# B3zaleel/draco-sharp

Measured on AMD Instinct MI355X. Metric: decoded_meshes_per_sec, higher is better.
Workload: dtype int32

## Files before the change

### draco-sharp_amd/csrc/dsa_kernels.h

```cpp
#pragma once
#include <hip/hip_runtime.h>
#include <stdint.h>

#include "dsa_common.h"
#include "dsa_locate.h"
#ifdef DSA_EXPERIMENTS
#include "dsa_lanes.h"
#else
#define LN_FLAG_SYMBOLS 1u
#define LN_FLAG_PREDICT 2u
#define LN_FLAG_OCT 8u
namespace dsa { namespace lanes {
__device__ __forceinline__ bool ln_sym_eligible(const AttrDesc &, const MeshLayout &, uint32_t, uint32_t) { return false; }
__device__ __forceinline__ bool ln_oct_eligible(const AttrDesc &, uint32_t) { return false; }
} }
#endif

#ifndef DSA_CHAIN_PRIO
#define DSA_CHAIN_PRIO 3
#endif

namespace dsa {

__device__ __forceinline__ uint32_t cnext(uint32_t c) { return (c % 3u == 2u) ? c - 2u : c + 1u; }
// ... 9 lines not shown
#define SYM_WIDE 0x800u
#define SYM_EARLY_ONLY 0x100u
#define SYM_LATE_ONLY 0x200u
#define SYM_CORNER 0x1000u
#define PRED_FRONT 0x10000u
#define PRED_BEHIND 0x20000u
__device__ __forceinline__ bool att_behind_tables(const AttrDesc &a) { return a.corner_data != 0 || a.late_located != 0; }
__device__ __forceinline__ bool att_is_late(const AttrDesc &a) { return (a.have_scheme && a.pred_kind != 0) || att_behind_tables(a); }
#define PW_FLAG 4u
#define LATE_HANDOFF 0x40000u
__device__ __forceinline__ void late_handoff(uint8_t *arena, const MeshLayout &L, MeshDesc *D, uint32_t ai, uint32_t flags, uint32_t bit);
__device__ __forceinline__ bool pred_filtered(const AttrDesc &a, uint32_t flags) {
  return ((flags & PRED_FRONT) && att_behind_tables(a)) || ((flags & PRED_BEHIND) && !att_behind_tables(a));
}
__device__ __forceinline__ bool sym_filtered(const AttrDesc &a, uint32_t flags) {
  if (att_behind_tables(a)) return !(flags & SYM_CORNER);
  if (flags & SYM_CORNER) return true;
  const bool late = a.have_scheme && a.pred_kind != 0;
  return ((flags & SYM_EARLY_ONLY) && late) || ((flags & SYM_LATE_ONLY) && !late);
}
__device__ __forceinline__ uint64_t clk() { return __builtin_amdgcn_s_memtime(); }
__device__ __forceinline__ uint64_t realclk() { return __builtin_amdgcn_s_memrealtime(); }
__device__ __forceinline__ uint32_t leading_lanes(bool pred) { uint64_t m = ~__ballot(pred); return m ? (uint32_t)__builtin_ctzll(m) : 64u; }
#define WAIT_VM0() __builtin_amdgcn_s_waitcnt(0x0F70)

template <int CTRL>
__device__ __forceinline__ uint32_t dpp_mov(uint32_t x) { return (uint32_t)__builtin_amdgcn_update_dpp(0, (int)x, CTRL, 0xF, 0xF, false); }
__device__ __forceinline__ uint32_t lane_prev(uint32_t x) { return dpp_mov<0x138>(x); }
template <class Op>
__device__ __forceinline__ uint32_t wave_incl_scan(uint32_t x, Op op) {
  const uint32_t lane = lane_id(), rl = lane & 15u;
  uint32_t t;
  t = dpp_mov<0x111>(x); if (rl >= 1) x = op(t, x);
  t = dpp_mov<0x112>(x); if (rl >= 2) x = op(t, x);
  t = dpp_mov<0x114>(x); if (rl >= 4) x = op(t, x);
  t = dpp_mov<0x118>(x); if (rl >= 8) x = op(t, x);
  t = dpp_mov<0x142>(x); if ((lane & 31u) >= 16) x = op(t, x);
  t = dpp_mov<0x143>(x); if (lane >= 32) x = op(t, x);
  return x;
}
__device__ __forceinline__ uint32_t wave_excl_scan(uint32_t v, uint32_t *total) {
  const uint32_t x = wave_incl_scan(v, [](uint32_t a, uint32_t b) { return a + b; });
  *total = rdlane(x, 63);
  return x - v;
}

template <bool CP> struct Rec;
struct FaceIds { uint32_t v0, v1, v2, o0, o1, o2; };
template <> struct Rec<false> {
  static constexpr uint32_t WORDS = 8;
  struct Raw { uint4 v, o; };
  static __device__ __forceinline__ Raw load(const uint32_t *frec, uint32_t f) { Raw r; r.v = ((const uint4 *)frec)[(size_t)f * 2]; r.o = ((const uint4 *)frec)[(size_t)f * 2 + 1]; return r; }
  static __device__ __forceinline__ Raw none() { Raw r; r.v = make_uint4(0, 0, 0, 0); r.o = make_uint4(DSA_INVALID, DSA_INVALID, DSA_INVALID, 0); return r; }
  static __device__ __forceinline__ uint32_t sel3(uint32_t k, uint32_t x, uint32_t y, uint32_t z) { return k == 0 ? x : (k == 1 ? y : z); }
  static __device__ __forceinline__ uint32_t vertex(const Raw &r, uint32_t k) { return sel3(k, r.v.x, r.v.y, r.v.z); }
  static __device__ __forceinline__ uint32_t opp(const Raw &r, uint32_t k) { return sel3(k, r.o.x, r.o.y, r.o.z); }
  static __device__ __forceinline__ uint32_t get_v(const uint32_t *frec, uint32_t c) { return frec[fv_idx(c)]; }
  static __device__ __forceinline__ uint32_t get_o(const uint32_t *frec, uint32_t c) { return frec[fo_idx(c)]; }
  static __device__ __forceinline__ uint32_t get_o_plain(const uint32_t *frec, uint32_t c) { return frec[fo_idx(c)]; }
  static __device__ __forceinline__ void set_v(uint32_t *frec, uint32_t c, uint32_t val) { frec[fv_idx(c)] = val; }
  static __device__ __forceinline__ void link(uint32_t *frec, uint32_t c, uint32_t val) { frec[fo_idx(c)] = val; }
  static __device__ __forceinline__ void link_lds(uint32_t *stage, uint32_t c_rel, uint32_t val) { stage[fo_idx(c_rel)] = val; }
  static __device__ __forceinline__ void store(uint32_t *frec, uint32_t f, const FaceIds &x) {
    ((uint4 *)frec)[(size_t)f * 2] = make_uint4(x.v0, x.v1, x.v2, 0u); ((uint4 *)frec)[(size_t)f * 2 + 1] = make_uint4(x.o0, x.o1, x.o2, 0u);
  }
  static __device__ __forceinline__ void store_lds(uint32_t *stage, uint32_t slot, const FaceIds &x) {
    *(uint4 *)&stage[slot * 8] = make_uint4(x.v0, x.v1, x.v2, 0u); *(uint4 *)&stage[slot * 8 + 4] = make_uint4(x.o0, x.o1, x.o2, 0u);
  }
  static __device__ __forceinline__ uint4 vertices_of(const uint32_t *frec, uint32_t f) { return ((const uint4 *)frec)[(size_t)f * 2]; }
};
template <> struct Rec<true> {
  static constexpr uint32_t WORDS = 4;
  static constexpr uint32_t M = 0x1FFFFFu;
  struct Raw { uint64_t v, o; };
  static __device__ __forceinline__ uint64_t pack(uint32_t a, uint32_t b, uint32_t c) { return (uint64_t)(a & M) | ((uint64_t)(b & M) << 21) | ((uint64_t)(c & M) << 42); }
  static __device__ __forceinline__ uint32_t field(uint64_t w, uint32_t k) { return (uint32_t)((int32_t)((uint32_t)(w >> (21u * k)) << 11) >> 11); }
  static __device__ __forceinline__ Raw load(const uint32_t *frec, uint32_t f) { const uint4 q = ((const uint4 *)frec)[f]; Raw r; r.v = (uint64_t)q.x | ((uint64_t)q.y << 32); r.o = (uint64_t)q.z | ((uint64_t)q.w << 32); return r; }
  static __device__ __forceinline__ Raw none() { Raw r; r.v = 0; r.o = ~0ull; return r; }
  static __device__ __forceinline__ uint32_t vertex(const Raw &r, uint32_t k) { return field(r.v, k); }
  static __device__ __forceinline__ uint32_t opp(const Raw &r, uint32_t k) { return field(r.o, k); }
  static __device__ __forceinline__ uint32_t get_v(const uint32_t *frec, uint32_t c) { return field(((const uint64_t *)frec)[(size_t)(c >> 2) * 2], c & 3u); }
  static __device__ __forceinline__ uint32_t get_o(const uint32_t *frec, uint32_t c) {
    return field(__hip_atomic_load((const unsigned long long *)frec + (size_t)(c >> 2) * 2 + 1, __ATOMIC_RELAXED, __HIP_MEMORY_SCOPE_AGENT), c & 3u);
  }
  static __device__ __forceinline__ uint32_t get_o_plain(const uint32_t *frec, uint32_t c) { return field(((const uint64_t *)frec)[(size_t)(c >> 2) * 2 + 1], c & 3u); }
  static __device__ __forceinline__ void set_v(uint32_t *frec, uint32_t c, uint32_t val) {
    uint64_t *w = (uint64_t *)frec + (size_t)(c >> 2) * 2;
    const uint32_t sh = 21u * (c & 3u);
    *w = (*w & ~((uint64_t)M << sh)) | ((uint64_t)(val & M) << sh);
  }
  static __device__ __forceinline__ void link(uint32_t *frec, uint32_t c, uint32_t val) {
    const uint32_t sh = 21u * (c & 3u);
    atomicAnd((unsigned long long *)frec + (size_t)(c >> 2) * 2 + 1, ((unsigned long long)(val & M) << sh) | ~((unsigned long long)M << sh));
  }
  static __device__ __forceinline__ void link_lds(uint32_t *stage, uint32_t c_rel, uint32_t val) {
    const uint32_t sh = 21u * (c_rel & 3u);
    atomicAnd((unsigned long long *)stage + (size_t)(c_rel >> 2) * 2 + 1, ((unsigned long long)(val & M) << sh) | ~((unsigned long long)M << sh));
  }
  static __device__ __forceinline__ uint4 quad(const FaceIds &x) { const uint64_t v = pack(x.v0, x.v1, x.v2), o = pack(x.o0, x.o1, x.o2); return make_uint4((uint32_t)v, (uint32_t)(v >> 32), (uint32_t)o, (uint32_t)(o >> 32)); }
  static __device__ __forceinline__ void store(uint32_t *frec, uint32_t f, const FaceIds &x) { ((uint4 *)frec)[f] = quad(x); }
  static __device__ __forceinline__ void store_lds(uint32_t *stage, uint32_t slot, const FaceIds &x) { *(uint4 *)&stage[slot * 4] = quad(x); }
  static __device__ __forceinline__ uint4 vertices_of(const uint32_t *frec, uint32_t f) {
    const uint64_t v = ((const uint64_t *)frec)[(size_t)f * 2];
    return make_uint4(field(v, 0), field(v, 1), field(v, 2), 0u);
  }
};
__device__ __forceinline__ uint32_t k_next(uint32_t k) { return k == 2u ? 0u : k + 1u; }
__device__ __forceinline__ uint32_t k_prev(uint32_t k) { return k == 0u ? 2u : k - 1u; }

__device__ __forceinline__ uint8_t *seam_block(uint8_t *arena, const MeshLayout &L, const SeamLayout &g, uint32_t d) {
  return arena + L.seam + g.data + (uint64_t)d * g.data_stride;
}
__device__ __forceinline__ const uint32_t *att_para(uint8_t *arena, const MeshLayout &L, const MeshDesc *D, const AttrDesc &a) {
  if (a.corner_data == 0) return (const uint32_t *)(arena + L.para);
  const SeamLayout g = seam_layout(L.cap_faces, L.cap_vertices, D->num_att_data, L.rec_compact != 0);
  return (const uint32_t *)(seam_block(arena, L, g, (uint32_t)a.corner_data - 1u) + g.para);
}


template <bool TOGGLE>
__device__ __forceinline__ uint32_t rabs_block_to_words(const Rabs &rb, uint32_t count, uint32_t *words) {
  uint32_t state = rb.state, left = rb.off, first = DSA_INVALID;
  const uint32_t p = rb.p;
  const uintptr_t a0 = (uintptr_t)rb.buf + (left ? left - 1u : 0u);
  const uint32_t *wp = (const uint32_t *)(a0 & ~(uintptr_t)3);
  uint32_t sh = (uint32_t)(a0 & 3u) * 8u;
  uint32_t cur = wp[0], nxt = wp[-1];
  uint32_t word = 0, last = 1;
  for (uint32_t i = 0; i < count; ++i) {
    if (state < 4096u && left > 0u) {
      state = state * 256u + ((cur >> sh) & 255u);
// ... 851 lines not shown
  uint32_t F, NV, cap_entries, expect;
  int att_data;
};
__device__ __forceinline__ TravIO trav_position(uint8_t *arena, const MeshLayout &L, const MeshDesc *D) {
  TravIO io;
  io.frec = (const uint32_t *)(arena + L.frec); io.d2c = (uint32_t *)(arena + L.d2c); io.v2d = (int32_t *)(arena + L.v2d);
  io.fvis = arena + L.fvis; io.vflag = arena + L.vvis; io.stack = (uint32_t *)(arena + L.fstamp); io.para = (uint32_t *)(arena + L.para);
  io.F = D->num_faces; io.NV = D->num_vertices; io.cap_entries = L.cap_vertices; io.expect = D->num_enc_vertices; io.att_data = -1;
  return io;
}
__device__ __forceinline__ TravIO trav_attribute(uint8_t *arena, const MeshLayout &L, const MeshDesc *D, uint32_t d) {
  const SeamLayout g = seam_layout(L.cap_faces, L.cap_vertices, D->num_att_data, L.rec_compact != 0);
  uint8_t *blk = seam_block(arena, L, g, d);
  TravIO io;
  io.frec = (const uint32_t *)(blk + g.rec); io.d2c = (uint32_t *)(blk + g.d2c); io.v2d = (int32_t *)(blk + g.v2d);
  io.fvis = blk + g.fvis; io.vflag = blk + g.vflag; io.stack = (uint32_t *)(blk + g.stack); io.para = (uint32_t *)(blk + g.para);
  io.F = D->num_faces; io.NV = D->seam_nv[d]; io.cap_entries = 3u * L.cap_faces; io.expect = D->seam_nv[d]; io.att_data = (int)d;
  return io;
}
template <bool CP>
__device__ __forceinline__ void traverse_wave(uint8_t *arena, const MeshLayout &L, MeshDesc *D, const TravIO &io, uint32_t fuse_operands, unsigned long long *sh_tf,
                                              unsigned long long *sh_tv, uint32_t *sh_hist) {
  typedef Rec<CP> R;
  typedef typename R::Raw Raw;
  if (status_of(D) != ST_OK || D->encoder_type == 0 || D->general) return;
  const uint32_t *frec = io.frec;
  uint32_t *d2c = io.d2c;
  int32_t *v2d = io.v2d;
  uint8_t *fvis = io.fvis;
  uint8_t *vflag = io.vflag;
  const uint32_t F = uni(io.F), NV = uni(io.NV), cap_entries = uni(io.cap_entries), expect = uni(io.expect);
  const bool position = io.att_data < 0;
  uint32_t *stack = io.stack;
  const uint32_t stack_cap = F;
  const uint32_t lane = lane_id();
  const uint64_t t_start = clk(), r_start = realclk();

  uint32_t count = 0, sp = 0, f_scan = 0;
  uint32_t run_id = 0;
  bool have_prog = false, prog_lin = false;
  uint32_t p_a = 0, p_an = 0, p_b = 0, p_ta = 0, p_tb = 0, p_la = 0, p_rb = 0;
  uint32_t dir = 0, hist_strikes = 0;
  uint32_t backoff = 0;
  uint32_t fail_streak = 0;
  uint32_t window = WAVE, side1 = WAVE, side2 = WAVE;
  uint32_t n_run = 0, n_run_faces = 0, n_scalar = 0, n_fail = 0, n_fast = 0;
  bool failed = false;
  bool have_rec = false, have_state = false, must_scalar = false, have2 = false;
  bool no_hist = false;
  uint32_t c_v = 0, c_rc = 0, c_lc = 0, c_bits = 0;
  uint32_t c2_v = 0, c2_rc = 0, c2_lc = 0, c2_bits = 0;
#ifdef DSA_TRAV_PROFILE
  uint64_t tp_acc[6] = {0, 0, 0, 0, 0, 0}, tp_last = clk();
  uint32_t np_fast_hit = 0, np_dep = 0, np_head = 0, np_hist = 0, np_lin = 0, np_hand = 0;
#define TPROF(slot_) { const uint64_t t_ = clk(); tp_acc[slot_] += t_ - tp_last; tp_last = t_; }
#define TCOUNT(x_) ++x_
#else
#define TPROF(slot_)
#define TCOUNT(x_)
#endif
#define TR_FAIL(site) { if (lane == 0) fail(D, ST_INVALID, (site)); failed = true; break; }
#define VISIT_SCALAR(v_, c_, fl_) { if (lane == 0) { vflag[v_] = (uint8_t)((fl_) | 1u); d2c[count] = (c_); v2d[v_] = (int32_t)count; } ++count; }
  auto corner_ok = [&](uint32_t c) -> bool { return c < 4 * F && (c & 3u) != 3u; };

  for (;;) {
    if (sp == 0) {
      uint32_t found = DSA_INVALID;
      while (f_scan < F) {
        uint32_t f = f_scan + lane;
        uint64_t m = __ballot(f < F && fvis[f] == 0);
        if (m) { found = f_scan + (uint32_t)__builtin_ctzll(m); break; }
        f_scan += WAVE;
      }
      if (found == DSA_INVALID) break;
      f_scan = found;
      const uint32_t corner = 4 * found;
      if (lane == 0) stack[0] = corner;
      sp = 1;
      const uint4 vv = R::vertices_of(frec, found);
      const uint32_t nv = uni(vv.y), pv = uni(vv.z);
      if (nv >= NV || pv >= NV) TR_FAIL(300);
      { uint32_t uni_flag = uni((uint32_t)vflag[nv]); if (!(uni_flag & 1u)) { if (count >= cap_entries) TR_FAIL(302); VISIT_SCALAR(nv, corner + 1, uni_flag); } }
      WAIT_VM0();
      { uint32_t uni_flag = uni((uint32_t)vflag[pv]); if (!(uni_flag & 1u)) { if (count >= cap_entries) TR_FAIL(302); VISIT_SCALAR(pv, corner + 2, uni_flag); } }
      WAIT_VM0();
    }
    uint32_t corner = uni(stack[sp - 1]);
    have_prog = false; have_rec = false; have_state = false; must_scalar = false; have2 = false;
    if (corner == DSA_INVALID || corner >= 4 * F || uni((uint32_t)fvis[corner >> 2])) { --sp; continue; }

    for (;;) {
      uint32_t face = corner >> 2;
      uint32_t v = 0, rc = 0, lc = 0, bits = 0;
      bool have_kids = false;
      uint32_t kr_v = 0, kr_rc = 0, kr_lc = 0, kl_v = 0, kl_rc = 0, kl_lc = 0;
      uint32_t kind = 0;
      bool lin = false;
      (void)lin;
      uint32_t a = 0, b = 0, tipA = 0, lcA = DSA_INVALID, tipB = 0, rcB = DSA_INVALID, lcB = DSA_INVALID;
      uint32_t marks = 0x0000011Eu;
#define fA_before (marks & 1u)
#define fB_before ((marks >> 1) & 1u)
#define fR_before ((marks >> 2) & 1u)
#define fL_before ((marks >> 3) & 1u)
#define fLA_before ((marks >> 4) & 1u)
#define flA ((marks >> 8) & 3u)
#define flB ((marks >> 16) & 3u)
#define TR_MARKS(fa_, fb_, fr_, fl_, fla_, ta_, tb_) (((fa_) ? 1u : 0u) | ((fb_) ? 2u : 0u) | ((fr_) ? 4u : 0u) | ((fl_) ? 8u : 0u) | ((fla_) ? 16u : 0u) | (((ta_) & 3u) << 8) | (((tb_) & 3u) << 16))
      bool pair_ok = false;
      uint32_t len = 0;

      if (have_prog && backoff == 0) { kind = 1; lin = prog_lin; }
      else {
        Raw rb0 = R::none();
        bool have_seed = false;
        if (have_rec) { v = c_v; rc = c_rc; lc = c_lc; }
        else {
          const Raw r0 = R::load(frec, face);
          const uint32_t kc0 = corner & 3u;
          v = uni(R::vertex(r0, kc0)); rc = uni(R::opp(r0, k_next(kc0))); lc = uni(R::opp(r0, k_prev(kc0)));
        }
        if (v >= NV || (rc != DSA_INVALID && !corner_ok(rc)) || (lc != DSA_INVALID && !corner_ok(lc))) TR_FAIL(301);
        if (have_state) bits = c_bits;
        else {
          const uint32_t tip_flag = vflag[v];
          const uint32_t side_r = rc != DSA_INVALID ? (uint32_t)fvis[rc >> 2] : 1u, side_l = lc != DSA_INVALID ? (uint32_t)fvis[lc >> 2] : 1u;
          Raw rl0 = R::none();
          if (rc != DSA_INVALID) { rb0 = R::load(frec, rc >> 2); have_seed = true; }
          if (lc != DSA_INVALID) rl0 = R::load(frec, lc >> 2);
          have_kids = true;
          { const uint32_t kr = rc & 3u, kl = lc & 3u;
            kr_v = uni(R::vertex(rb0, kr)); kr_rc = uni(R::opp(rb0, k_next(kr))); kr_lc = uni(R::opp(rb0, k_prev(kr)));
            kl_v = uni(R::vertex(rl0, kl)); kl_rc = uni(R::opp(rl0, k_next(kl))); kl_lc = uni(R::opp(rl0, k_prev(kl))); }
          const uint32_t uf = uni(tip_flag);
          const bool rdone = rc == DSA_INVALID || (rc >> 2) == face || uni(side_r) != 0;
          const bool ldone = lc == DSA_INVALID || (lc >> 2) == face || uni(side_l) != 0;
          bits = ((uf & 1u) ? 0u : 1u) | (uf & 2u) | (rdone ? 4u : 0u) | (ldone ? 8u : 0u);
          TCOUNT(np_head);
        }
        have_rec = false; have_state = false;
        const bool moves_right = (bits & 3u) == 1u || ((bits & 12u) == 8u);
        if (moves_right && backoff == 0 && !must_scalar && rc != DSA_INVALID) {
          if (!have_seed) rb0 = R::load(frec, rc >> 2);
          const uint32_t kb0 = rc & 3u;
          const uint32_t tB0 = uni(R::vertex(rb0, kb0)), rB0 = uni(R::opp(rb0, k_next(kb0))), a1 = uni(R::opp(rb0, k_prev(kb0)));
          const uint32_t d1 = a1 - corner;
          const uint32_t e = dir & 3u;
          const bool hm = !no_hist && d1 != 0u && corner_ok(a1) && uni(sh_hist[8 * e]) == d1;
          if (hm) {
            const uint32_t s_b = uni(sh_hist[8 * e + 1]), s_ta = uni(sh_hist[8 * e + 2]), s_tb = uni(sh_hist[8 * e + 3]), s_la = uni(sh_hist[8 * e + 4]), s_rb = uni(sh_hist[8 * e + 5]);
            p_a = corner + lane * d1; p_an = p_a + d1; p_b = rc + lane * s_b; p_ta = v + lane * s_ta; p_tb = tB0 + lane * s_tb;
            p_la = lc == DSA_INVALID ? DSA_INVALID : lc + lane * s_la; p_rb = rB0 == DSA_INVALID ? DSA_INVALID : rB0 + lane * s_rb;
            kind = 2; lin = true;
            TCOUNT(np_hist);
          } else {
            kind = 3;
            auto opp_prev_of = [&](uint32_t b1) -> uint32_t { return corner_ok(b1) ? uni(R::get_o_plain(frec, qprev(b1))) : DSA_INVALID; };
            auto opp_next_of = [&](uint32_t c) -> uint32_t { return corner_ok(c) ? uni(R::get_o_plain(frec, qnext(c))) : DSA_INVALID; };
            const uint32_t a0 = corner;
            const uint32_t a2 = opp_prev_of(opp_next_of(a1));
            const uint32_t d2 = a2 - a1, ddh = d2 - d1;
            const uint32_t exact = corner_ok(a2) ? 3u : (corner_ok(a1) ? 2u : 1u);
            uint32_t lq = lane;
            asm volatile("" : "+v"(lq));
            a = lane == 0 ? a0 : lane == 1 ? a1 : lane == 2 ? a2 : a2 + (lane - 2u) * (d2 + ddh) + ddh * ((lq - 2u) * (lq - 3u) / 2u);
            bool a_ok = lane < window && corner_ok(a) && (lane < exact || exact == 3);
            Raw ra = R::none(), rb = R::none();
            if (a_ok) ra = R::load(frec, a >> 2);
            const uint32_t ka = a & 3u;
            tipA = R::vertex(ra, ka); b = R::opp(ra, k_next(ka)); lcA = R::opp(ra, k_prev(ka));
            const bool b_ok = a_ok && corner_ok(b) && tipA < NV && (lcA == DSA_INVALID || corner_ok(lcA));
            if (b_ok) rb = R::load(frec, b >> 2);
            const uint32_t kb = b & 3u;
            tipB = R::vertex(rb, kb); rcB = R::opp(rb, k_next(kb)); lcB = R::opp(rb, k_prev(kb));
            const uint32_t next_a = b_ok ? lcB : DSA_INVALID;
            {
              const uint32_t prev_next = lane_prev(next_a);
              a_ok = a_ok && (lane == 0 || prev_next == a);
            }
            len = leading_lanes(a_ok);
            pair_ok = lane < len && b_ok && tipB < NV && corner_ok(lcB) && (rcB == DSA_INVALID || corner_ok(rcB));
            if (pair_ok) {
              const uint32_t m0 = lane == 0 ? 0u : fvis[a >> 2], m4 = lcA != DSA_INVALID ? fvis[lcA >> 2] : 1u, m1 = fvis[b >> 2];
              const uint32_t m2 = rcB != DSA_INVALID ? fvis[rcB >> 2] : 1u, m3 = fvis[lcB >> 2], ta = vflag[tipA], tb = vflag[tipB];
              marks = TR_MARKS(m0, m1, m2, m3, m4, ta, tb);
            }
            TCOUNT(np_dep);
          }
        } else if (backoff) --backoff;
        must_scalar = false;
        TPROF(1);
      }

      if (kind == 1 || kind == 2) {
        ++n_fast;
        a = p_a;
        const bool a_ok = lane < window && corner_ok(a);
        const bool bp_ok = a_ok && corner_ok(p_b);
        Raw ra = R::none(), rb = R::none();
        if (a_ok) ra = R::load(frec, a >> 2);
        if (bp_ok) rb = R::load(frec, p_b >> 2);
        if (bp_ok) {
          const uint32_t m0 = lane == 0 ? 0u : fvis[a >> 2], m1 = fvis[p_b >> 2], m4 = corner_ok(p_la) ? fvis[p_la >> 2] : 1u;
          const uint32_t m2 = corner_ok(p_rb) ? fvis[p_rb >> 2] : 1u, m3 = corner_ok(p_an) ? fvis[p_an >> 2] : 1u;
          const uint32_t ta = p_ta < NV ? vflag[p_ta] : 1u, tb = p_tb < NV ? vflag[p_tb] : 1u;
          marks = TR_MARKS(m0, m1, m2, m3, m4, ta, tb);
        }
        const uint32_t ka = a & 3u, kb = p_b & 3u;
        tipA = R::vertex(ra, ka); b = R::opp(ra, k_next(ka)); lcA = R::opp(ra, k_prev(ka));
        tipB = R::vertex(rb, kb); rcB = R::opp(rb, k_next(kb)); lcB = R::opp(rb, k_prev(kb));
        const bool match = bp_ok && b == p_b && tipA == p_ta && lcA == p_la && tipB == p_tb && rcB == p_rb && lcB == p_an &&
                           tipA < NV && tipB < NV && corner_ok(lcB) && (lcA == DSA_INVALID || corner_ok(lcA)) && (rcB == DSA_INVALID || corner_ok(rcB));
        len = leading_lanes(match);
        pair_ok = lane < len;
        if (kind == 1) {
          v = rdlane(tipA, 0); rc = rdlane(b, 0); lc = rdlane(lcA, 0);
          if (v >= NV || (rc != DSA_INVALID && !corner_ok(rc)) || (lc != DSA_INVALID && !corner_ok(lc))) TR_FAIL(301);
        }
        TPROF(0);
      } else if (kind == 3) { TPROF(2); }

      if (kind) {
        const uint32_t fa = a >> 2, fb = b >> 2;
        const uint32_t keyN = 2 * lane, keyL = 2 * lane + 1;
        uint32_t sfa = TR_NONE, sfb = TR_NONE, sta = TR_NONE, stb = TR_NONE, srf = TR_NONE, slf = TR_NONE, sla = TR_NONE;
        int32_t fa0, fas, fad, fb0, fbs, fbd, ta0, tas, tad, tb0, tbs, tbd;
        bool arith;
        {
          const uint32_t tri = lane * (lane - 1u) / 2u;
          const bool two = len >= 2, three = len >= 3;
          auto fit = [&](uint32_t x, int32_t &q0, int32_t &qs, int32_t &qd) {
            const uint32_t x0 = rdlane(x, 0), x1 = rdlane(x, 1), x2 = rdlane(x, 2);
            q0 = (int32_t)x0; qs = two ? (int32_t)(x1 - x0) : 1; qd = three ? (int32_t)((x2 - x1) - (x1 - x0)) : 0;
          };
          auto mono = [&](int32_t s_, int32_t d_) -> bool {
            const int32_t last = s_ + d_ * (int32_t)(two ? len - 2u : 0u);
            return s_ != 0 && last != 0 && ((s_ ^ last) >= 0) && d_ > -(1 << 24) && d_ < (1 << 24);
          };
          int32_t a0, as_, ad, b0, bs_, bd;
          fit(a, a0, as_, ad); fit(b, b0, bs_, bd); fit(tipA, ta0, tas, tad); fit(tipB, tb0, tbs, tbd);
          arith = ((as_ | ad | bs_ | bd) & 3) == 0 && mono(as_, ad) && mono(bs_, bd) && mono(tas, tad) && mono(tbs, tbd);
          if (arith && kind == 3)
            arith = __ballot(lane < len && (a != (uint32_t)a0 + lane * (uint32_t)as_ + (uint32_t)ad * tri || b != (uint32_t)b0 + lane * (uint32_t)bs_ + (uint32_t)bd * tri ||
                                            tipA != (uint32_t)ta0 + lane * (uint32_t)tas + (uint32_t)tad * tri || tipB != (uint32_t)tb0 + lane * (uint32_t)tbs + (uint32_t)tbd * tri)) == 0;
          fa0 = a0 >> 2; fas = as_ >> 2; fad = ad >> 2; fb0 = b0 >> 2; fbs = bs_ >> 2; fbd = bd >> 2;
        }
        if (arith) {
          TCOUNT(np_lin);
          const float iA = 1.0f / (float)fas, iB = 1.0f / (float)fbs, iTA = 1.0f / (float)tas, iTB = 1.0f / (float)tbs;
          auto pos_in = [&](uint32_t X, int32_t first, int32_t step, int32_t dd, float inv, uint32_t odd) -> uint32_t {
            if (dd == 0) {
              const int32_t d = (int32_t)X - first;
              const int32_t j = (int32_t)__builtin_rintf((float)d * inv);
              return (j >= 0 && (uint32_t)j < len && j * step == d) ? 2u * (uint32_t)j + odd : TR_NONE;
            }
            int32_t j = 0;
#pragma unroll
            for (int32_t bit = 32; bit >= 1; bit >>= 1) {
              const int32_t t = j + bit;
              const int32_t qt = first + t * step + dd * (t * (t - 1) / 2);
              if ((uint32_t)t < len && (step > 0 ? qt <= (int32_t)X : qt >= (int32_t)X)) j = t;
            }
            return first + j * step + dd * (j * (j - 1) / 2) == (int32_t)X ? 2u * (uint32_t)j + odd : TR_NONE;
          };
          auto face_pos = [&](uint32_t X) -> uint32_t { const uint32_t x = pos_in(X, fa0, fas, fad, iA, 0u), y = pos_in(X, fb0, fbs, fbd, iB, 1u); return x < y ? x : y; };
          auto tip_pos = [&](uint32_t X) -> uint32_t { const uint32_t x = pos_in(X, ta0, tas, tad, iTA, 0u), y = pos_in(X, tb0, tbs, tbd, iTB, 1u); return x < y ? x : y; };
          if (pair_ok) {
            sfa = face_pos(fa); sfb = face_pos(fb);
            if (!(flA & 1u)) sta = tip_pos(tipA);
            if (!(flB & 1u)) stb = tip_pos(tipB);
            if (rcB != DSA_INVALID && fR_before == 0) srf = face_pos(rcB >> 2);
            if (fL_before == 0) slf = face_pos(lcB >> 2);
            if (lcA != DSA_INVALID && fLA_before == 0 && flA != 0) sla = face_pos(lcA >> 2);
          }
        } else {
          if (++run_id >= 0x00FFFFF0u) {
            __syncthreads();
            for (uint32_t i = lane; i < TR_SLOTS; i += WAVE) { sh_tf[i] = 0; sh_tv[i] = 0; }
            __syncthreads();
            run_id = 1;
          }
          const uint32_t run_tag = 0x00FFFFFFu - run_id;
          auto tbl_insert = [&](unsigned long long *t, uint32_t id, uint32_t pos) {
            const unsigned long long want = ((unsigned long long)run_tag << 40) | ((unsigned long long)id << 8) | pos;
            uint32_t sl = (id * 2654435761u) >> (32 - TR_SLOT_BITS);
            for (;;) {
              const unsigned long long cur = __hip_atomic_load(&t[sl], __ATOMIC_RELAXED, __HIP_MEMORY_SCOPE_WORKGROUP);
              if ((uint32_t)(cur >> 40) != run_tag) { if (atomicCAS(&t[sl], cur, want) == cur) break; continue; }
              if ((uint32_t)(cur >> 8) == id) { atomicMin(&t[sl], want); break; }
              sl = (sl + 1) & (TR_SLOTS - 1);
            }
          };
          auto tbl_lookup = [&](unsigned long long *t, uint32_t id) -> uint32_t {
            uint32_t sl = (id * 2654435761u) >> (32 - TR_SLOT_BITS);
            for (uint32_t probes = 0; probes < TR_SLOTS; ++probes) {
              const unsigned long long cur = __hip_atomic_load(&t[sl], __ATOMIC_RELAXED, __HIP_MEMORY_SCOPE_WORKGROUP);
              if ((uint32_t)(cur >> 40) != run_tag) return TR_NONE;
              if ((uint32_t)(cur >> 8) == id) return (uint32_t)(cur & 0xFFu);
              sl = (sl + 1) & (TR_SLOTS - 1);
            }
            return TR_NONE;
          };
          if (pair_ok) {
            tbl_insert(sh_tf, fa, 2 * lane); tbl_insert(sh_tf, fb, 2 * lane + 1);
            if (!(flA & 1u)) tbl_insert(sh_tv, tipA, 2 * lane);
            if (!(flB & 1u)) tbl_insert(sh_tv, tipB, 2 * lane + 1);
          }
          __syncthreads();
          if (pair_ok) {
            sfa = tbl_lookup(sh_tf, fa); sfb = tbl_lookup(sh_tf, fb);
            if (!(flA & 1u)) sta = tbl_lookup(sh_tv, tipA);
            if (!(flB & 1u)) stb = tbl_lookup(sh_tv, tipB);
            if (rcB != DSA_INVALID && fR_before == 0) srf = tbl_lookup(sh_tf, rcB >> 2);
            if (fL_before == 0) slf = tbl_lookup(sh_tf, lcB >> 2);
            if (lcA != DSA_INVALID && fLA_before == 0 && flA != 0) sla = tbl_lookup(sh_tf, lcA >> 2);
          }
        }
        bool good = false, newA = false, newB = false;
        uint32_t hand = 0;
        if (pair_ok) {
          newA = !(flA & 1u) && sta == keyN;
          const bool la_done = lcA == DSA_INVALID || (lcA >> 2) == fa || fLA_before != 0 || sla < keyN;
          const bool x_ok = fA_before == 0 && sfa == keyN && ((newA && !(flA & 2u)) || la_done);
          newB = !(flB & 1u) && stb == keyL;
          const bool r_done = rcB == DSA_INVALID || (rcB >> 2) == fb || fR_before != 0 || srf < keyL;
          const bool l_open = (lcB >> 2) != fb && fL_before == 0 && !(slf < keyL);
          const bool y_ok = fB_before == 0 && sfb == keyL && !(newB && !(flB & 2u)) && r_done && l_open;
          good = x_ok && y_ok;
// ... 12 lines not shown
        TPROF(3);
        const uint64_t kmask = K >= 64 ? ~0ull : ((1ull << K) - 1ull);
        const uint64_t mA = __ballot(newA) & kmask, mB = __ballot(newB) & kmask;
        const uint32_t made = (uint32_t)__popcll(mA) + (uint32_t)__popcll(mB);
        const bool retire = K >= 1 && count + made <= cap_entries;
        const uint32_t win_used = window;
        have_prog = false;
        if (kind == 2) {
          if (K == len && len <= 2 && len < window) { if (++hist_strikes >= 2) { if (lane == 0) sh_hist[8 * (dir & 3u)] = 0; hist_strikes = 0; } }
          else if (K >= 3) hist_strikes = 0;
        }
        if (retire) {
          if (lane < K) {
            const uint64_t lt = (1ull << lane) - 1ull;
            const uint32_t posA = count + (uint32_t)__popcll(mA & lt) + (uint32_t)__popcll(mB & lt);
            fvis[fa] = 1; fvis[fb] = 1;
            if (newA) { vflag[tipA] = (uint8_t)(flA | 1u); d2c[posA] = a; v2d[tipA] = (int32_t)posA; }
            if (newB) { const uint32_t posB = posA + (newA ? 1u : 0u); vflag[tipB] = (uint8_t)(flB | 1u); d2c[posB] = b; v2d[tipB] = (int32_t)posB; }
          }
          const uint32_t nxt = rdlane(lcB, K - 1);
          count += made;
          if (K >= 3) {
            const uint32_t aK1 = rdlane(a, K - 1), aK2 = rdlane(a, K - 2), aK3 = rdlane(a, K - 3);
            const uint32_t s1 = nxt - aK1, s0 = aK1 - aK2, sm = aK2 - aK3;
            const uint32_t a_d = (s1 - s0 == s0 - sm) ? s1 - s0 : 0u, a_s = s1 + a_d;
            uint32_t any_d = a_d | (s1 ^ s0);
            const bool cont = K == window;
            const uint32_t l1 = lane + 1u, tri1 = l1 * (l1 + 1u) / 2u;
            if (cont) {
              uint32_t lq = lane;
              asm volatile("" : "+v"(lq));
              p_a = nxt + lane * a_s + a_d * (lq * (lq - 1u) / 2u); p_an = nxt + l1 * a_s + a_d * ((lq + 1u) * lq / 2u);
            }
            uint32_t st_b, st_ta, st_tb, st_la, st_rb;
#define TR_PROG(q_, p_, st_) { const uint32_t x1 = rdlane(q_, K - 1), x2 = rdlane(q_, K - 2), x3 = rdlane(q_, K - 3); \
                               const uint32_t t0 = x1 - x2, qd = t0 - (x2 - x3); any_d |= qd; st_ = t0; if (cont) p_ = x1 + l1 * t0 + qd * tri1; }
            TR_PROG(b, p_b, st_b); TR_PROG(tipA, p_ta, st_ta); TR_PROG(tipB, p_tb, st_tb); TR_PROG(lcA, p_la, st_la); TR_PROG(rcB, p_rb, st_rb);
#undef TR_PROG
            const bool linear = any_d == 0 && (s0 & 3u) == 0 && (st_b & 3u) == 0 && s0 != 0 && st_b != 0 && st_ta != 0 && st_tb != 0;
            have_prog = cont; prog_lin = linear;
            if (linear && kind == 3) {
              const uint32_t e = dir & 3u;
              if (lane == 0) { sh_hist[8 * e] = s0; sh_hist[8 * e + 1] = st_b; sh_hist[8 * e + 2] = st_ta; sh_hist[8 * e + 3] = st_tb; sh_hist[8 * e + 4] = st_la; sh_hist[8 * e + 5] = st_rb; }
            }
          }
          corner = nxt;
          face = corner >> 2;
          have_kids = false;
          n_run += 1; n_run_faces += 2 * K;
          fail_streak = 0; no_hist = false;
          if ((fuse_operands & 2u) && K < window && len > K) { side2 = side1; side1 = K; const uint32_t m = (side1 > side2 ? side1 : side2) + 4; window = m < WAVE ? m : WAVE; }
          else window = WAVE;
          if (kind != 3) TCOUNT(np_fast_hit);
          TPROF(4);
          if (K >= win_used) continue;
          if (K < len) ++dir;
        } else {
          ++n_fail;
          if (kind == 3) { backoff = fail_streak < 3 ? fail_streak : 3; ++fail_streak; }
          if (kind == 2) no_hist = true;
        }
        {
          const uint32_t h_lane = retire ? K : 0u;
          const uint32_t h = (h_lane < win_used && h_lane < len) ? rdlane(hand, h_lane) : 0u;
          if (h & 1u) {
            v = rdlane(tipA, h_lane); rc = rdlane(b, h_lane); lc = rdlane(lcA, h_lane);
            if (h & 512u) {
              bits = ((h & 2u) ? 1u : 0u) | ((h & 4u) ? 2u : 0u) | ((h & 8u) ? 4u : 0u) | ((h & 16u) ? 8u : 0u);
              have2 = (h & 1024u) != 0;
              c2_v = rdlane(tipB, h_lane); c2_rc = rdlane(rcB, h_lane); c2_lc = rdlane(lcB, h_lane);
              c2_bits = ((h & 32u) ? 1u : 0u) | ((h & 64u) ? 2u : 0u) | ((h & 128u) ? 4u : 0u) | ((h & 256u) ? 8u : 0u);
              TCOUNT(np_hand);
            } else { have_rec = true; c_v = v; c_rc = rc; c_lc = lc; must_scalar = true; continue; }
          } else if (kind != 3 || retire) {
            const bool rec_ok = h_lane < WAVE && h_lane < win_used && (kind != 3 || h_lane < len);
            if (rec_ok && rdlane(a, h_lane) == corner) { have_rec = true; c_v = rdlane(tipA, h_lane); c_rc = rdlane(b, h_lane); c_lc = rdlane(lcA, h_lane); }
            must_scalar = retire && h_lane < len;
            continue;
          }
        }
      }
      ++n_scalar;
      no_hist = false;
      if (lane == 0) fvis[face] = 1;
      bool went_right = false;
      if (bits & 1u) {
        if (count >= cap_entries) TR_FAIL(302);
        VISIT_SCALAR(v, corner, bits & 2u);
        if (!(bits & 2u)) {
          if (rc == DSA_INVALID) TR_FAIL(303);
          corner = rc;
          went_right = true;
        }
      }
      bool went_left = false;
      if (!went_right) {
        if (bits & 4u) {
          if (bits & 8u) { --sp; TPROF(5); break; }
          corner = lc;
          went_left = true;
        } else {
          if (bits & 8u) { corner = rc; went_right = true; }
          else {
            if (sp >= stack_cap) TR_FAIL(304);
            if (lane == 0) { stack[sp - 1] = lc; stack[sp] = rc; }
            ++sp;
            TPROF(5);
            break;
          }
        }
      }
      if (went_right && have2) { have_rec = true; have_state = true; c_v = c2_v; c_rc = c2_rc; c_lc = c2_lc; c_bits = c2_bits; }
      else if (have_kids && went_right) { have_rec = true; c_v = kr_v; c_rc = kr_rc; c_lc = kr_lc; }
      else if (have_kids && went_left) { have_rec = true; c_v = kl_v; c_rc = kl_rc; c_lc = kl_lc; }
      have2 = false;
      TPROF(5);
    }
    if (failed) break;
  }
  if (failed) return;
  if (lane == 0 && !position) { if (count != expect) fail(D, ST_INVALID, 305); }
  if (lane == 0 && position) {
    D->num_entries = count;
    D->dbg[5] = n_fail; D->dbg[6] = (uint32_t)(clk() - t_start);
    D->dbg[16] = (uint32_t)r_start; D->dbg[17] = (uint32_t)(realclk() - r_start);
    D->dbg[7] = n_run; D->dbg[8] = n_run_faces; D->dbg[9] = n_scalar; D->dbg[3] = n_fast;
#ifdef DSA_TRAV_PROFILE
    for (int i = 0; i < 5; ++i) D->dbg[10 + (i < 3 ? i : i + 5)] = (uint32_t)(tp_acc[i] >> 4);
    D->dbg[0] = (uint32_t)(tp_acc[5] >> 4); D->dbg[1] = np_fast_hit; D->dbg[2] = np_dep; D->dbg[4] = np_head; D->dbg[13] = np_hist; D->dbg[14] = np_lin; D->dbg[15] = np_hand;
#endif
    if (count != expect) fail(D, ST_INVALID, 305);
  }
  if ((fuse_operands & 1u) && count == expect) {
    WAIT_VM0();
    __threadfence_block();
    uint32_t *para = io.para;
    for (uint32_t p0 = 0; p0 < count; p0 += 4 * WAVE) {
      uint32_t en[4], ep[4], eo[4];
#pragma unroll
      for (int u = 0; u < 4; ++u) {
        const uint32_t p = p0 + u * WAVE + lane;
        para_operands_flat<CP>(p < count ? p : 0u, frec, d2c, v2d, F, NV, en[u], ep[u], eo[u]);
      }
#pragma unroll
      for (int u = 0; u < 4; ++u) {
        const uint32_t p = p0 + u * WAVE + lane;
        if (p < count) { Triple t; t.a = en[u]; t.b = ep[u]; t.c = eo[u]; *(Triple *)(para + 3 * (size_t)p) = t; }
      }
    }
  }
  if (position && !D->seam_fast && count == expect && NV) {
    WAIT_VM0();
    __threadfence_block();
    const uint32_t *vrank = (const uint32_t *)(arena + L.vrank);
    const uint32_t na = uni(D->num_attributes), npts = uni(D->num_points);
    for (uint32_t v0 = 0; v0 < NV; v0 += 4 * WAVE) {
      int32_t e[4];
      uint32_t point[4];
#pragma unroll
      for (int u = 0; u < 4; ++u) {
        const uint32_t v = v0 + u * WAVE + lane, vc = v < NV ? v : NV - 1;
        e[u] = v < NV ? v2d[vc] : -1;
        point[u] = vrank[vc];
      }
#pragma unroll
      for (int u = 0; u < 4; ++u)
        if (e[u] >= 0 && point[u] < npts)
          for (uint32_t ai = 0; ai < na; ++ai) ((uint32_t *)(arena + L.map[ai]))[point[u]] = (uint32_t)e[u];
    }
  }
#undef TR_FAIL
#undef VISIT_SCALAR
#undef TPROF
#undef TCOUNT
#undef fA_before
#undef fB_before
#undef fR_before
#undef fL_before
#undef fLA_before
#undef flA
#undef flB
#undef TR_MARKS
}

__global__ __launch_bounds__(WAVE) void k_traverse(uint8_t *arena, const MeshLayout *layouts, MeshDesc *descs, uint32_t n, uint32_t fuse_operands) {
  __shared__ unsigned long long sh_tf[TR_SLOTS], sh_tv[TR_SLOTS];
  __shared__ uint32_t sh_hist[TR_HIST_WORDS];
  for (uint32_t i = threadIdx.x; i < TR_SLOTS; i += WAVE) { sh_tf[i] = 0; sh_tv[i] = 0; }
  if (threadIdx.x < TR_HIST_WORDS) sh_hist[threadIdx.x] = 0;
  __syncthreads();
  __builtin_amdgcn_s_setprio(DSA_CHAIN_PRIO);
  const uint32_t mesh = blockIdx.x;
  if (mesh >= n) return;
  if (status_of(&descs[mesh]) != ST_OK) return;
  const TravIO io = trav_position(arena, layouts[mesh], &descs[mesh]);
  if (layouts[mesh].rec_compact) traverse_wave<true>(arena, layouts[mesh], &descs[mesh], io, fuse_operands, sh_tf, sh_tv, sh_hist);
  else traverse_wave<false>(arena, layouts[mesh], &descs[mesh], io, fuse_operands, sh_tf, sh_tv, sh_hist);
}

extern __shared__ __attribute__((aligned(16))) uint32_t sh_chain[];
__global__ __launch_bounds__(WAVE, 8) void k_chain(uint8_t *arena, const MeshLayout *layouts, MeshDesc *descs, uint32_t n, uint32_t fuse_operands) {
  uint32_t *sh = sh_chain;
  static_assert(CN_LDS_WORDS * 4 >= 2 * TR_SLOTS * 8 + TR_HIST_WORDS * 4, "the traversal's tables reuse the connectivity's LDS");
  __builtin_amdgcn_s_setprio(DSA_CHAIN_PRIO);
  const uint32_t mesh = blockIdx.x;
  if (mesh >= n) return;
  const MeshLayout &L = layouts[mesh];
  MeshDesc *D = &descs[mesh];
  const bool compact = uni(L.rec_compact) != 0;
  uint32_t *sh_rec = sh + CN_STAGE * 8, *sh_win = sh_rec + CN_REC_BLOCKS * 64 * 2, *sh_ctx = sh_win + CN_WIN;
  if (!compact) connectivity_wave<false, false>(arena, L, D, sh, sh_rec, sh_win, sh_ctx);
  else if (uni((uint32_t)D->traversal_type) == 2u) connectivity_wave<true, true>(arena, L, D, sh, sh_rec, sh_win, sh_ctx);
  else connectivity_wave<true, false>(arena, L, D, sh, sh_rec, sh_win, sh_ctx);
  __builtin_amdgcn_fence(__ATOMIC_SEQ_CST, "agent");
  __syncthreads();
  unsigned long long *sh_tf = (unsigned long long *)sh, *sh_tv = sh_tf + TR_SLOTS;
  uint32_t *sh_hist = sh + 2 * TR_SLOTS * 2;
  for (uint32_t i = threadIdx.x; i < TR_SLOTS; i += WAVE) { sh_tf[i] = 0; sh_tv[i] = 0; }
  if (threadIdx.x < TR_HIST_WORDS) sh_hist[threadIdx.x] = 0;
  __syncthreads();
  if (status_of(D) != ST_OK) return;
  const TravIO io = trav_position(arena, L, D);
  if (compact) traverse_wave<true>(arena, L, D, io, fuse_operands, sh_tf, sh_tv, sh_hist);
  else traverse_wave<false>(arena, L, D, io, fuse_operands, sh_tf, sh_tv, sh_hist);
  if ((fuse_operands & 1u) && (fuse_operands & 8u) && status_of(D) == ST_OK) {
    const uint32_t na = uni(D->num_attributes);
    for (uint32_t ai = 0; ai < na && ai < DSA_MAX_ATT; ++ai) late_handoff(arena, L, D, ai, PW_FLAG | LATE_HANDOFF, 2u);
// ... 1491 lines not shown
```

Before: 102,700.

## Hoist traversal loads unconditionally and drop arithmetic-progression detection path

Makes the face-record and visited-flag loads in the traversal step unconditional, using clamped indices and select masks, so they can issue together instead of behind branches. Removes the arithmetic-progression fit and closed-form position lookup, so every run goes through the hashed slot-table path. Adds optional compile-time switches that disable the fast, history and dependent paths, plus profile counters. In exchange it issues some redundant loads at index 0, and runs that the closed-form path used to handle now pay the hashing cost.

```diff
diff --git a/draco-sharp_amd/csrc/dsa_kernels.h b/draco-sharp_amd/csrc/dsa_kernels.h
--- a/draco-sharp_amd/csrc/dsa_kernels.h
+++ b/draco-sharp_amd/csrc/dsa_kernels.h
@@ -85,6 +85,7 @@
   struct Raw { uint4 v, o; };
   static __device__ __forceinline__ Raw load(const uint32_t *frec, uint32_t f) { Raw r; r.v = ((const uint4 *)frec)[(size_t)f * 2]; r.o = ((const uint4 *)frec)[(size_t)f * 2 + 1]; return r; }
   static __device__ __forceinline__ Raw none() { Raw r; r.v = make_uint4(0, 0, 0, 0); r.o = make_uint4(DSA_INVALID, DSA_INVALID, DSA_INVALID, 0); return r; }
+  static __device__ __forceinline__ Raw or_none(bool ok, const Raw &x) { return ok ? x : none(); }
   static __device__ __forceinline__ uint32_t sel3(uint32_t k, uint32_t x, uint32_t y, uint32_t z) { return k == 0 ? x : (k == 1 ? y : z); }
   static __device__ __forceinline__ uint32_t vertex(const Raw &r, uint32_t k) { return sel3(k, r.v.x, r.v.y, r.v.z); }
   static __device__ __forceinline__ uint32_t opp(const Raw &r, uint32_t k) { return sel3(k, r.o.x, r.o.y, r.o.z); }
@@ -110,6 +111,7 @@
   static __device__ __forceinline__ uint32_t field(uint64_t w, uint32_t k) { return (uint32_t)((int32_t)((uint32_t)(w >> (21u * k)) << 11) >> 11); }
   static __device__ __forceinline__ Raw load(const uint32_t *frec, uint32_t f) { const uint4 q = ((const uint4 *)frec)[f]; Raw r; r.v = (uint64_t)q.x | ((uint64_t)q.y << 32); r.o = (uint64_t)q.z | ((uint64_t)q.w << 32); return r; }
   static __device__ __forceinline__ Raw none() { Raw r; r.v = 0; r.o = ~0ull; return r; }
+  static __device__ __forceinline__ Raw or_none(bool ok, const Raw &x) { Raw r; r.v = ok ? x.v : 0ull; r.o = ok ? x.o : ~0ull; return r; }
   static __device__ __forceinline__ uint32_t vertex(const Raw &r, uint32_t k) { return field(r.v, k); }
   static __device__ __forceinline__ uint32_t opp(const Raw &r, uint32_t k) { return field(r.o, k); }
   static __device__ __forceinline__ uint32_t get_v(const uint32_t *frec, uint32_t c) { return field(((const uint64_t *)frec)[(size_t)(c >> 2) * 2], c & 3u); }
@@ -1067,12 +1069,14 @@
   uint32_t c2_v = 0, c2_rc = 0, c2_lc = 0, c2_bits = 0;
 #ifdef DSA_TRAV_PROFILE
   uint64_t tp_acc[6] = {0, 0, 0, 0, 0, 0}, tp_last = clk();
-  uint32_t np_fast_hit = 0, np_dep = 0, np_head = 0, np_hist = 0, np_lin = 0, np_hand = 0;
+  uint32_t np_fast_hit = 0, np_dep = 0, np_head = 0, np_hist = 0, np_lin = 0, np_hand = 0, np_pairs1 = 0, np_pairs2 = 0;
 #define TPROF(slot_) { const uint64_t t_ = clk(); tp_acc[slot_] += t_ - tp_last; tp_last = t_; }
 #define TCOUNT(x_) ++x_
+#define TADD(x_, n_) x_ += (n_)
 #else
 #define TPROF(slot_)
 #define TCOUNT(x_)
+#define TADD(x_, n_)
 #endif
 #define TR_FAIL(site) { if (lane == 0) fail(D, ST_INVALID, (site)); failed = true; break; }
 #define VISIT_SCALAR(v_, c_, fl_) { if (lane == 0) { vflag[v_] = (uint8_t)((fl_) | 1u); d2c[count] = (c_); v2d[v_] = (int32_t)count; } ++count; }
@@ -1125,6 +1129,9 @@
       bool pair_ok = false;
       uint32_t len = 0;
 
+#ifdef DSA_TRAV_NO_FAST
+      have_prog = false;
+#endif
       if (have_prog && backoff == 0) { kind = 1; lin = prog_lin; }
       else {
         Raw rb0 = R::none();
@@ -1138,11 +1145,13 @@
         if (v >= NV || (rc != DSA_INVALID && !corner_ok(rc)) || (lc != DSA_INVALID && !corner_ok(lc))) TR_FAIL(301);
         if (have_state) bits = c_bits;
         else {
-          const uint32_t tip_flag = vflag[v];
-          const uint32_t side_r = rc != DSA_INVALID ? (uint32_t)fvis[rc >> 2] : 1u, side_l = lc != DSA_INVALID ? (uint32_t)fvis[lc >> 2] : 1u;
-          Raw rl0 = R::none();
-          if (rc != DSA_INVALID) { rb0 = R::load(frec, rc >> 2); have_seed = true; }
-          if (lc != DSA_INVALID) rl0 = R::load(frec, lc >> 2);
+          const bool r_ok = rc != DSA_INVALID, l_ok = lc != DSA_INVALID;
+          const uint32_t fr = r_ok ? rc >> 2 : 0u, fl = l_ok ? lc >> 2 : 0u;
+          const uint32_t tip_flag = vflag[v], side_r0 = fvis[fr], side_l0 = fvis[fl];
+          rb0 = R::or_none(r_ok, R::load(frec, fr));
+          const Raw rl0 = R::or_none(l_ok, R::load(frec, fl));
+          have_seed = r_ok;
+          const uint32_t side_r = r_ok ? side_r0 : 1u, side_l = l_ok ? side_l0 : 1u;
           have_kids = true;
           { const uint32_t kr = rc & 3u, kl = lc & 3u;
             kr_v = uni(R::vertex(rb0, kr)); kr_rc = uni(R::opp(rb0, k_next(kr))); kr_lc = uni(R::opp(rb0, k_prev(kr)));
@@ -1161,6 +1170,9 @@
           const uint32_t tB0 = uni(R::vertex(rb0, kb0)), rB0 = uni(R::opp(rb0, k_next(kb0))), a1 = uni(R::opp(rb0, k_prev(kb0)));
           const uint32_t d1 = a1 - corner;
           const uint32_t e = dir & 3u;
+#ifdef DSA_TRAV_NO_HIST
+          no_hist = true;
+#endif
           const bool hm = !no_hist && d1 != 0u && corner_ok(a1) && uni(sh_hist[8 * e]) == d1;
           if (hm) {
             const uint32_t s_b = uni(sh_hist[8 * e + 1]), s_ta = uni(sh_hist[8 * e + 2]), s_tb = uni(sh_hist[8 * e + 3]), s_la = uni(sh_hist[8 * e + 4]), s_rb = uni(sh_hist[8 * e + 5]);
@@ -1168,7 +1180,11 @@
             p_la = lc == DSA_INVALID ? DSA_INVALID : lc + lane * s_la; p_rb = rB0 == DSA_INVALID ? DSA_INVALID : rB0 + lane * s_rb;
             kind = 2; lin = true;
             TCOUNT(np_hist);
-          } else {
+          }
+#ifdef DSA_TRAV_NO_DEP
+          else { }
+#else
+          else {
             kind = 3;
             auto opp_prev_of = [&](uint32_t b1) -> uint32_t { return corner_ok(b1) ? uni(R::get_o_plain(frec, qprev(b1))) : DSA_INVALID; };
             auto opp_next_of = [&](uint32_t c) -> uint32_t { return corner_ok(c) ? uni(R::get_o_plain(frec, qnext(c))) : DSA_INVALID; };
@@ -1196,12 +1212,14 @@
             len = leading_lanes(a_ok);
             pair_ok = lane < len && b_ok && tipB < NV && corner_ok(lcB) && (rcB == DSA_INVALID || corner_ok(rcB));
             if (pair_ok) {
-              const uint32_t m0 = lane == 0 ? 0u : fvis[a >> 2], m4 = lcA != DSA_INVALID ? fvis[lcA >> 2] : 1u, m1 = fvis[b >> 2];
-              const uint32_t m2 = rcB != DSA_INVALID ? fvis[rcB >> 2] : 1u, m3 = fvis[lcB >> 2], ta = vflag[tipA], tb = vflag[tipB];
-              marks = TR_MARKS(m0, m1, m2, m3, m4, ta, tb);
+              const bool la_ok = lcA != DSA_INVALID, rb_ok = rcB != DSA_INVALID;
+              const uint32_t m0 = fvis[a >> 2], m4 = fvis[la_ok ? lcA >> 2 : 0u], m1 = fvis[b >> 2];
+              const uint32_t m2 = fvis[rb_ok ? rcB >> 2 : 0u], m3 = fvis[lcB >> 2], ta = vflag[tipA], tb = vflag[tipB];
+              marks = TR_MARKS(lane == 0 ? 0u : m0, m1, rb_ok ? m2 : 1u, m3, la_ok ? m4 : 1u, ta, tb);
             }
             TCOUNT(np_dep);
           }
+#endif
         } else if (backoff) --backoff;
         must_scalar = false;
         TPROF(1);
@@ -1212,15 +1230,14 @@
         a = p_a;
         const bool a_ok = lane < window && corner_ok(a);
         const bool bp_ok = a_ok && corner_ok(p_b);
-        Raw ra = R::none(), rb = R::none();
-        if (a_ok) ra = R::load(frec, a >> 2);
-        if (bp_ok) rb = R::load(frec, p_b >> 2);
-        if (bp_ok) {
-          const uint32_t m0 = lane == 0 ? 0u : fvis[a >> 2], m1 = fvis[p_b >> 2], m4 = corner_ok(p_la) ? fvis[p_la >> 2] : 1u;
-          const uint32_t m2 = corner_ok(p_rb) ? fvis[p_rb >> 2] : 1u, m3 = corner_ok(p_an) ? fvis[p_an >> 2] : 1u;
-          const uint32_t ta = p_ta < NV ? vflag[p_ta] : 1u, tb = p_tb < NV ? vflag[p_tb] : 1u;
-          marks = TR_MARKS(m0, m1, m2, m3, m4, ta, tb);
-        }
+        const bool la_ok = corner_ok(p_la), rb_ok = corner_ok(p_rb), an_ok = corner_ok(p_an), ta_ok = p_ta < NV, tb_ok = p_tb < NV;
+        const uint32_t fa_l = a_ok ? a >> 2 : 0u, fb_l = bp_ok ? p_b >> 2 : 0u;
+        const Raw ra0 = R::load(frec, fa_l), rb1 = R::load(frec, fb_l);
+        const uint32_t m0 = fvis[fa_l], m1 = fvis[fb_l], m4 = fvis[la_ok ? p_la >> 2 : 0u];
+        const uint32_t m2 = fvis[rb_ok ? p_rb >> 2 : 0u], m3 = fvis[an_ok ? p_an >> 2 : 0u];
+        const uint32_t ta = vflag[ta_ok ? p_ta : 0u], tb = vflag[tb_ok ? p_tb : 0u];
+        const Raw ra = R::or_none(a_ok, ra0), rb = R::or_none(bp_ok, rb1);
+        if (bp_ok) marks = TR_MARKS(lane == 0 ? 0u : m0, m1, rb_ok ? m2 : 1u, an_ok ? m3 : 1u, la_ok ? m4 : 1u, ta_ok ? ta : 1u, tb_ok ? tb : 1u);
         const uint32_t ka = a & 3u, kb = p_b & 3u;
         tipA = R::vertex(ra, ka); b = R::opp(ra, k_next(ka)); lcA = R::opp(ra, k_prev(ka));
         tipB = R::vertex(rb, kb); rcB = R::opp(rb, k_next(kb)); lcB = R::opp(rb, k_prev(kb));
@@ -1239,56 +1256,7 @@
         const uint32_t fa = a >> 2, fb = b >> 2;
         const uint32_t keyN = 2 * lane, keyL = 2 * lane + 1;
         uint32_t sfa = TR_NONE, sfb = TR_NONE, sta = TR_NONE, stb = TR_NONE, srf = TR_NONE, slf = TR_NONE, sla = TR_NONE;
-        int32_t fa0, fas, fad, fb0, fbs, fbd, ta0, tas, tad, tb0, tbs, tbd;
-        bool arith;
         {
-          const uint32_t tri = lane * (lane - 1u) / 2u;
-          const bool two = len >= 2, three = len >= 3;
-          auto fit = [&](uint32_t x, int32_t &q0, int32_t &qs, int32_t &qd) {
-            const uint32_t x0 = rdlane(x, 0), x1 = rdlane(x, 1), x2 = rdlane(x, 2);
-            q0 = (int32_t)x0; qs = two ? (int32_t)(x1 - x0) : 1; qd = three ? (int32_t)((x2 - x1) - (x1 - x0)) : 0;
-          };
-          auto mono = [&](int32_t s_, int32_t d_) -> bool {
-            const int32_t last = s_ + d_ * (int32_t)(two ? len - 2u : 0u);
-            return s_ != 0 && last != 0 && ((s_ ^ last) >= 0) && d_ > -(1 << 24) && d_ < (1 << 24);
-          };
-          int32_t a0, as_, ad, b0, bs_, bd;
-          fit(a, a0, as_, ad); fit(b, b0, bs_, bd); fit(tipA, ta0, tas, tad); fit(tipB, tb0, tbs, tbd);
-          arith = ((as_ | ad | bs_ | bd) & 3) == 0 && mono(as_, ad) && mono(bs_, bd) && mono(tas, tad) && mono(tbs, tbd);
-          if (arith && kind == 3)
-            arith = __ballot(lane < len && (a != (uint32_t)a0 + lane * (uint32_t)as_ + (uint32_t)ad * tri || b != (uint32_t)b0 + lane * (uint32_t)bs_ + (uint32_t)bd * tri ||
-                                            tipA != (uint32_t)ta0 + lane * (uint32_t)tas + (uint32_t)tad * tri || tipB != (uint32_t)tb0 + lane * (uint32_t)tbs + (uint32_t)tbd * tri)) == 0;
-          fa0 = a0 >> 2; fas = as_ >> 2; fad = ad >> 2; fb0 = b0 >> 2; fbs = bs_ >> 2; fbd = bd >> 2;
-        }
-        if (arith) {
-          TCOUNT(np_lin);
-          const float iA = 1.0f / (float)fas, iB = 1.0f / (float)fbs, iTA = 1.0f / (float)tas, iTB = 1.0f / (float)tbs;
-          auto pos_in = [&](uint32_t X, int32_t first, int32_t step, int32_t dd, float inv, uint32_t odd) -> uint32_t {
-            if (dd == 0) {
-              const int32_t d = (int32_t)X - first;
-              const int32_t j = (int32_t)__builtin_rintf((float)d * inv);
-              return (j >= 0 && (uint32_t)j < len && j * step == d) ? 2u * (uint32_t)j + odd : TR_NONE;
-            }
-            int32_t j = 0;
-#pragma unroll
-            for (int32_t bit = 32; bit >= 1; bit >>= 1) {
-              const int32_t t = j + bit;
-              const int32_t qt = first + t * step + dd * (t * (t - 1) / 2);
-              if ((uint32_t)t < len && (step > 0 ? qt <= (int32_t)X : qt >= (int32_t)X)) j = t;
-            }
-            return first + j * step + dd * (j * (j - 1) / 2) == (int32_t)X ? 2u * (uint32_t)j + odd : TR_NONE;
-          };
-          auto face_pos = [&](uint32_t X) -> uint32_t { const uint32_t x = pos_in(X, fa0, fas, fad, iA, 0u), y = pos_in(X, fb0, fbs, fbd, iB, 1u); return x < y ? x : y; };
-          auto tip_pos = [&](uint32_t X) -> uint32_t { const uint32_t x = pos_in(X, ta0, tas, tad, iTA, 0u), y = pos_in(X, tb0, tbs, tbd, iTB, 1u); return x < y ? x : y; };
-          if (pair_ok) {
-            sfa = face_pos(fa); sfb = face_pos(fb);
-            if (!(flA & 1u)) sta = tip_pos(tipA);
-            if (!(flB & 1u)) stb = tip_pos(tipB);
-            if (rcB != DSA_INVALID && fR_before == 0) srf = face_pos(rcB >> 2);
-            if (fL_before == 0) slf = face_pos(lcB >> 2);
-            if (lcA != DSA_INVALID && fLA_before == 0 && flA != 0) sla = face_pos(lcA >> 2);
-          }
-        } else {
           if (++run_id >= 0x00FFFFF0u) {
             __syncthreads();
             for (uint32_t i = lane; i < TR_SLOTS; i += WAVE) { sh_tf[i] = 0; sh_tv[i] = 0; }
@@ -1407,6 +1375,8 @@
           if ((fuse_operands & 2u) && K < window && len > K) { side2 = side1; side1 = K; const uint32_t m = (side1 > side2 ? side1 : side2) + 4; window = m < WAVE ? m : WAVE; }
           else window = WAVE;
           if (kind != 3) TCOUNT(np_fast_hit);
+          if (kind == 1) TADD(np_pairs1, K);
+          if (kind == 2) TADD(np_pairs2, K);
           TPROF(4);
           if (K >= win_used) continue;
           if (K < len) ++dir;
@@ -1483,6 +1453,7 @@
 #ifdef DSA_TRAV_PROFILE
     for (int i = 0; i < 5; ++i) D->dbg[10 + (i < 3 ? i : i + 5)] = (uint32_t)(tp_acc[i] >> 4);
     D->dbg[0] = (uint32_t)(tp_acc[5] >> 4); D->dbg[1] = np_fast_hit; D->dbg[2] = np_dep; D->dbg[4] = np_head; D->dbg[13] = np_hist; D->dbg[14] = np_lin; D->dbg[15] = np_hand;
+    D->dbg[16] = np_pairs1; D->dbg[17] = np_pairs2;
 #endif
     if (count != expect) fail(D, ST_INVALID, 305);
   }
@@ -1528,6 +1499,7 @@
 #undef VISIT_SCALAR
 #undef TPROF
 #undef TCOUNT
+#undef TADD
 #undef fA_before
 #undef fB_before
 #undef fR_before
```

Result: faster. 108,700, median of 6 (+5.9%).
